# baaivision/Painter

Hardware: AMD Instinct MI355X
Metric: images/sec (896x448 pairs) ViT-L fwd+bwd (higher is better)
Workload: dtype bf16; 1 GPU; painter_vit_large_patch16_input896x448 bf16 batch=8/GPU fwd+bwd on 1xMI355X (BASELINE configs[1]); global_batch=8, image=896x448x3 stitched pair, mode=train (DropPath 0.1), parallelism=dp1, rccl_ranks=0, backend=n/a, grad_allreduce=n/a

## Files before the change

### include/painter_hip.h

```cpp
#ifndef PAINTER_HIP_H
#define PAINTER_HIP_H

#include <stdint.h>

#ifdef __cplusplus
extern "C" {
#endif

#ifndef __HIP__
typedef struct ihipStream_t* hipStream_t;
#endif

enum { PA_F32 = 0, PA_BF16 = 1 };
enum {
    PA_EPI_BIAS = 0,
    PA_EPI_BIAS_F32 = 1,
    PA_EPI_BIAS_GELU = 2,
    PA_EPI_BIAS_RESID = 3
};

#define PA_ABI_VERSION 8
int pa_abi_version(void);
int pa_debug_set(int which, int value);
int pa_debug_get(int which);

int pa_linear_fwd(int dtype, int epilogue, const void* x , int64_t ldx, const void* w ,
                  const float* bias , void* out, void* out2, int64_t ldo, const float* resid ,
                  const float* rowscale , int rows_per_sample, int M, int N, int K,
                  hipStream_t stream);
int pa_linear_fwd_skip(int dtype, int epilogue, const void* x, int64_t ldx, const void* w, const float* bias, void* out, void* out2,
                       int64_t ldo, const float* resid, const float* rowscale, int rows_per_sample, int M, int N, int K,
                       const float* rowskip, int skip_rows_per_sample, hipStream_t stream);
int pa_linear_pixshuf(int dtype, const void* x, int64_t ldx, const void* w , const float* bias,
                      void* out_nhwc, int batch, int Hp, int Wp, int P, int C, int K, hipStream_t stream);
int64_t pa_linear_dgrad_workspace_bytes(int M, int K);
int pa_linear_dgrad(int dtype, const void* dy , int64_t lddy, const void* w ,
                    const void* gelu_aux , void* dx , int64_t lddx, float* dx_colsum,
                    void* workspace, int M, int N, int K, hipStream_t stream);
int pa_linear_dgrad_skip(int dtype, const void* dy, int64_t lddy, const void* w, const void* gelu_aux, void* dx, int64_t lddx, float* dx_colsum,
                         void* workspace, int M, int N, int K, const float* rowskip , int skip_rows_per_sample,
                         hipStream_t stream);
int64_t pa_linear_wgrad_workspace_bytes(int dtype, int M, int N, int K);
int pa_linear_wgrad(int dtype, const void* dy , int64_t lddy, const void* x , int64_t ldx,
                    float* dw , void* workspace, int M, int N, int K, hipStream_t stream);
int64_t pa_colsum_workspace_bytes(int M, int N);
int pa_colsum(int dtype, const void* x , int64_t ld, int M, int N, float* out , void* workspace,
              hipStream_t stream);
int pa_slab_reduce(const float* in, float* out, int64_t n, int nz, int64_t stride, int accumulate, hipStream_t stream);

int pa_layernorm_fwd(int dtype, const float* x, int64_t ldx, const float* gamma, const float* beta, float eps,
                     void* y , int64_t ldy, float* mean, float* rstd,
                     int R, int D, hipStream_t stream);
int64_t pa_layernorm_bwd_workspace_bytes(int R, int D);
int pa_layernorm_bwd(int dtype, const void* dy, int64_t lddy, const float* x, int64_t ldx, const float* mean,
                     const float* rstd, const float* gamma, const float* dres, float* dx, int64_t lddx, void* dxT,
                     int64_t lddxT, const float* rowscale, int rows_per_sample, float* dgamma_dbeta, float* dxT_colsum,
                     void* workspace, int R, int D, hipStream_t stream);
// ... 250 lines not shown
```

### painter_amd/_lib.py

```python
import ctypes
import os
import re

HERE = os.path.dirname(os.path.abspath(__file__))
HEADER = os.path.join(os.path.dirname(HERE), "include", "painter_hip.h")
LIB_PATH = os.environ.get("PAINTER_AMD_LIB") or os.path.join(HERE, "lib", "libpainter_hip.so")

PA_F32, PA_BF16 = 0, 1
EPI_BIAS, EPI_BIAS_F32, EPI_BIAS_GELU, EPI_BIAS_RESID = 0, 1, 2, 3
(KNOB_G256_STAGGER, KNOB_G256_NOSTORE, KNOB_G256_ORDER, KNOB_WGRAD_TARGET, KNOB_G256_SHORT_TILES, KNOB_G256_ILV, KNOB_RELPOS_SPLITS,
 KNOB_ATTN3_FUSE, KNOB_ATTN_LIGHT_LAST, KNOB_CONV_WGRAD_GROUPS, KNOB_LN_BWD_VARIANT, KNOB_G256_PATCH, KNOB_G256_MIXED) = range(13)
KNOB_G256_MIXED_NFULL, KNOB_DROP_SKIP, KNOB_DECODER_ROWS, KNOB_COUNT = 14, 16, 17, 18

_CT = {"int": ctypes.c_int, "int64_t": ctypes.c_int64, "float": ctypes.c_float, "double": ctypes.c_double, "hipStream_t": ctypes.c_void_p}


def parse_header(path=HEADER):
    src = open(path).read()
    src = re.sub(r"/\*.*?\*/", " ", src, flags=re.S)
    src = re.sub(r"//[^\n]*", " ", src)
    protos = {}
    for m in re.finditer(r"\b(int64_t|int)\s+(pa_\w+)\s*\(([^)]*)\)\s*;", src):
        ret, name, args = m.group(1), m.group(2), m.group(3).strip()
        argtypes = []
        if args and args != "void":
            for a in args.split(","):
                a = a.strip()
                if "*" in a:
                    argtypes.append(ctypes.c_void_p)
                else:
                    t = a.replace("const", " ").split()[0]
                    argtypes.append(_CT[t])
        protos[name] = (_CT[ret], argtypes)
    return protos


class _Lib:
    def __init__(self):
        self._dll = None
        self._protos = parse_header()

    def load(self):
        if self._dll is None:
            if not os.path.exists(LIB_PATH):
                raise RuntimeError(
                    "painter_amd: %s is missing -- run `python -m painter_amd.build` (or __graft_entry__.build()). "
                    "There is no CPU / PyTorch fallback for the hot path." % LIB_PATH)
            import torch
            dll = ctypes.CDLL(LIB_PATH)
            for name, (ret, args) in self._protos.items():
                fn = getattr(dll, name)
                fn.restype = ret
                fn.argtypes = args
            want = int(re.search(r"#define\s+PA_ABI_VERSION\s+(\d+)", open(HEADER).read()).group(1))
            got = dll.pa_abi_version()
            if got != want:
                raise RuntimeError("painter_amd: %s has C ABI version %d, include/painter_hip.h declares %d -- rebuild it "
                                   "(python -m painter_amd.build --force)" % (LIB_PATH, got, want))
            self._dll = dll
        return self._dll

    def __getattr__(self, name):
        if name.startswith("_"):
            raise AttributeError(name)
        return getattr(self.load(), name)


lib = _Lib()


def check(err, what=""):
    if err != 0:
        raise RuntimeError("painter_hip: %s failed with hipError %d" % (what, err))
```

### painter_amd/csrc/common.h

```cpp
#pragma once
#include <hip/hip_runtime.h>
#include <stdint.h>
#include <cstdlib>

typedef __bf16 bf16;
typedef __attribute__((ext_vector_type(8))) __bf16 bf16x8;
typedef __attribute__((ext_vector_type(16))) float f32x16;

#define DEVI __device__ __forceinline__

template <typename T> struct TT;
template <> struct TT<float> {
    static constexpr int EPC = 4;
    static constexpr int BK = 32;
    static constexpr int KSTEPS = 2;
    static constexpr int SPF = 2;
    typedef uint4 Vec4;
};
template <> struct TT<bf16> {
    static constexpr int EPC = 8;
    static constexpr int BK = 64;
    static constexpr int KSTEPS = 4;
    static constexpr int SPF = 1;
    typedef uint2 Vec4;
// ... 51 lines not shown
    const uint32_t u = __builtin_bit_cast(uint32_t, v);
    const auto r = __builtin_amdgcn_permlane16_swap(u, u, false, false);
    return __builtin_bit_cast(float, (threadIdx.x & 16) ? r[0] : r[1]);
}
DEVI float lane_xor32(float v) {
    const uint32_t u = __builtin_bit_cast(uint32_t, v);
    const auto r = __builtin_amdgcn_permlane32_swap(u, u, false, false);
    return __builtin_bit_cast(float, (threadIdx.x & 32) ? r[0] : r[1]);
}
DEVI float quad_sum(float v) { v += lane_xor1(v); v += lane_xor2(v); return v; }
DEVI float row16_sum(float v) { v = quad_sum(v); v += lane_dpp<0x141>(v); v += lane_dpp<0x140>(v); return v; }
DEVI float wave_sum(float v) { v = row16_sum(v); v += lane_xor16(v); v += lane_xor32(v); return v; }
DEVI float wave_max(float v) {
    v = fmaxf(v, lane_xor1(v)); v = fmaxf(v, lane_xor2(v));
    v = fmaxf(v, lane_dpp<0x141>(v)); v = fmaxf(v, lane_dpp<0x140>(v));
    v = fmaxf(v, lane_xor16(v)); v = fmaxf(v, lane_xor32(v));
    return v;
}

enum Knob {
    KNOB_G256_STAGGER = 0,
    KNOB_G256_NOSTORE = 1,
    KNOB_G256_ORDER = 2,
    KNOB_WGRAD_TARGET = 3,
    KNOB_G256_SHORT_TILES = 4,
    KNOB_G256_ILV = 5,
    KNOB_RELPOS_SPLITS = 6,
    KNOB_ATTN3_FUSE = 7,
    KNOB_ATTN_LIGHT_LAST = 8,
    KNOB_CONV_WGRAD_GROUPS = 9,
    KNOB_LN_BWD_VARIANT = 10,
    KNOB_G256_PATCH = 11,
    KNOB_G256_MIXED = 12,
    KNOB_FREE_13 = 13,
    KNOB_G256_MIXED_NFULL = 14,
    KNOB_FREE_15 = 15,
    KNOB_DROP_SKIP = 16,
    KNOB_DECODER_ROWS = 17,
    KNOB_COUNT = 18
};
inline int g_knob[KNOB_COUNT] = {};
static inline bool drop_skip_on() {
    static const int env = [] { const char* v = getenv("PAINTER_AMD_DROP_SKIP"); return v ? atoi(v) : 1; }();
    return g_knob[KNOB_DROP_SKIP] == 1 ? false : (g_knob[KNOB_DROP_SKIP] == 2 ? true : env != 0);
}
static inline bool decoder_rows_on() {
    static const int env = [] { const char* v = getenv("PAINTER_AMD_DECODER_ROWS"); return v ? atoi(v) : 1; }();
    return g_knob[KNOB_DECODER_ROWS] == 1 ? false : (g_knob[KNOB_DECODER_ROWS] == 2 ? true : env != 0);
}

inline long long g_attn_counts[6] = {0, 0, 0, 0, 0, 0};

DEVI float gelu_f(float x) { return 0.5f * x * (1.0f + erff(x * 0.70710678118654752f)); }
DEVI float gelu_grad_f(float x) {
    const float cdf = 0.5f * (1.0f + erff(x * 0.70710678118654752f));
    const float pdf = 0.39894228040143268f * __expf(-0.5f * x * x);
    return cdf + x * pdf;
}

DEVI void gelu_parts(float x, float& cdf, float& pdf_unnorm) {
    const float z = fabsf(x) * 0.70710678118654752f;
    const float t = __builtin_amdgcn_rcpf(fmaf(0.3275911f, z, 1.0f));
    const float e = __builtin_amdgcn_exp2f(-0.72134752044448170f * x * x);
    float p = fmaf(1.061405429f, t, -1.453152027f);
    p = fmaf(p, t, 1.421413741f);
    p = fmaf(p, t, -0.284496736f);
    p = fmaf(p, t, 0.254829592f);
// ... 68 lines not shown
```

### painter_amd/csrc/gemm.hip

```cpp
#include <cstdlib>
#include "gemm_engine.h"
#include "gemm256.h"
#include "../../include/painter_hip.h"

template <typename OutT> struct EpiBias {
    OutT* out; size_t ldo; const float* bias; int M, N;
    DEVI void operator()(const f32x16 (&acc)[2][2], int ib, int jb, int lane, int) const {
        foreach_acc(acc, ib, jb, lane, [&](int i, int j, float v) {
            if (i < M && j < N) out[(size_t)i * ldo + j] = from_f<OutT>(v + (bias ? bias[j] : 0.f));
        });
    }
};
constexpr float G8_OFF = 0.13f, G8_SCALE = 255.f / 1.26f, G8_STEP = 1.26f / 255.f;
DEVI uint32_t g8_code(float g) { return min((uint32_t)fmaf(g, G8_SCALE, G8_OFF * G8_SCALE + 0.5f), 255u); }
DEVI float g8_value(uint32_t q) { return fmaf((float)q, G8_STEP, -G8_OFF); }
template <typename T> struct GeluAux { typedef T type; };
template <> struct GeluAux<bf16> { typedef unsigned char type; };
template <typename T> struct EpiBiasGelu {
    typename GeluAux<T>::type* aux; T* act; size_t ld; const float* bias; int M, N;
    DEVI void operator()(const f32x16 (&acc)[2][2], int ib, int jb, int lane, int) const {
        foreach_acc(acc, ib, jb, lane, [&](int i, int j, float v) {
            if (i < M && j < N) {
                const T p = from_f<T>(v + bias[j]);
                if constexpr (std::is_same<T, bf16>::value) {
// ... 173 lines not shown
    struct Row { uint2 p; };
    DEVI Col col(int) const { return Col{}; }
    DEVI Row row(int i, int j) const {
        Row r{make_uint2(0, 0)};
        if (i < M && j < N) r.p = *reinterpret_cast<const uint2*>(aux + (size_t)i * ld + j);
        return r;
    }
    DEVI void decode(const Row& r, float (&g)[8]) const {
#pragma unroll
        for (int e = 0; e < 8; ++e) g[e] = g8_value(((e < 4 ? r.p.x : r.p.y) >> (8 * (e & 3))) & 0xffu);
    }
    DEVI void store(int i, int j, float4 a, float4 b, const Col&, const Row& r, int) const {
        if (i >= M || j >= N) return;
        float g[8];
        decode(r, g);
        store8(out + (size_t)i * ld + j, make_float4(a.x * g[0], a.y * g[1], a.z * g[2], a.w * g[3]), make_float4(b.x * g[4], b.y * g[5], b.z * g[6], b.w * g[7]));
    }
};
struct Epi4DGeluCS : Epi4DGelu {
    float* part;
    DEVI void store_cs(int i, int j, float4 a, float4 b, const Col&, const Row& r, int, float (&cs)[8]) const {
        if (i >= M || j >= N) return;
        float g[8];
        decode(r, g);
        const uint4 pk = make_uint4(pack_bf16x2(a.x * g[0], a.y * g[1]), pack_bf16x2(a.z * g[2], a.w * g[3]),
                                    pack_bf16x2(b.x * g[4], b.y * g[5]), pack_bf16x2(b.z * g[6], b.w * g[7]));
        *reinterpret_cast<uint4*>(out + (size_t)i * ld + j) = pk;
        cs[0] = fmaf(a.x, g[0], cs[0]); cs[1] = fmaf(a.y, g[1], cs[1]); cs[2] = fmaf(a.z, g[2], cs[2]); cs[3] = fmaf(a.w, g[3], cs[3]);
        cs[4] = fmaf(b.x, g[4], cs[4]); cs[5] = fmaf(b.y, g[5], cs[5]); cs[6] = fmaf(b.z, g[6], cs[6]); cs[7] = fmaf(b.w, g[7], cs[7]);
    }
    DEVI void colsum_out(int prow, int j, const float (&cs)[8]) const {
        if (j >= N) return;
        float* o = part + (size_t)prow * N + j;
        *reinterpret_cast<float4*>(o) = make_float4(cs[0], cs[1], cs[2], cs[3]);
        *reinterpret_cast<float4*>(o + 4) = make_float4(cs[4], cs[5], cs[6], cs[7]);
    }
};
template <> struct g256::epi_colsum<Epi4DGeluCS> { static constexpr bool value = true; };
struct Epi4PixShuf {
    bf16* out; const float* bias; int Hp, Wp, P, C, M, N;
    typedef EpiCol8 Col;
    typedef EpiNone Row;
    DEVI Col col(int j) const { return load_col8(bias, j, N); }
    DEVI Row row(int, int) const { return Row{}; }
    DEVI void store(int i, int j, float4 a, float4 b, const Col& cc, const Row&, int) const {
        if (i >= M || j >= N) return;
        const int L = Hp * Wp;
        const int bb = i / L, l = i - bb * L, h = l / Wp, w = l - h * Wp;
        const int c = j % C, pq = j / C, q = pq % P, p = pq / P;
        const size_t y = (size_t)bb * Hp * P + h * P + p, x = (size_t)w * P + q;
        store8(out + (y * (size_t)(Wp * P) + x) * C + c, add4(a, cc.a), add4(b, cc.b));
    }
};
struct Epi4Slab {
    float* out; size_t ldo; size_t slab; int M, N;
    static constexpr int HI_OFF = 32;
    typedef EpiNone Col;
    typedef EpiNone Row;
    DEVI Col col(int) const { return Col{}; }
    DEVI Row row(int, int) const { return Row{}; }
    DEVI void store(int i, int j, float4 a, float4 b, const Col&, const Row&, int split) const {
        if (i >= M || j >= N) return;
        store44(out + (size_t)split * slab + (size_t)i * ldo + j, j, N, a, b);
    }
};

__global__ __launch_bounds__(256) void slab_reduce_kernel(const float* __restrict__ in, float* out, size_t n, int nz, size_t stride, int accumulate) {
    __shared__ float4 sh[16][17];
    const int cg = threadIdx.x & 15, zl = threadIdx.x >> 4;
    const size_t i = ((size_t)blockIdx.x * 16 + cg) * 4;
    float4 s = make_float4(0, 0, 0, 0);
    if (i < n) {
#pragma unroll 4
        for (int z = zl; z < nz; z += 16) {
            const float4 v = *reinterpret_cast<const float4*>(in + (size_t)z * stride + i);
            s.x += v.x; s.y += v.y; s.z += v.z; s.w += v.w;
        }
    }
    sh[zl][cg] = s;
    __syncthreads();
    if (zl == 0 && i < n) {
        float4 t = accumulate ? *reinterpret_cast<const float4*>(out + i) : make_float4(0, 0, 0, 0);
#pragma unroll
        for (int k = 0; k < 16; ++k) { const float4 v = sh[k][cg]; t.x += v.x; t.y += v.y; t.z += v.z; t.w += v.w; }
        *reinterpret_cast<float4*>(out + i) = t;
    }
}
__global__ void slab_reduce_wide_kernel(const float* __restrict__ in, float* out, size_t n, int nz, size_t stride, int accumulate) {
    const size_t i = ((size_t)blockIdx.x * blockDim.x + threadIdx.x) * 4;
    if (i >= n) return;
    float4 s = accumulate ? *reinterpret_cast<const float4*>(out + i) : make_float4(0, 0, 0, 0);
#pragma unroll 4
    for (int z = 0; z < nz; ++z) {
        const float4 v = *reinterpret_cast<const float4*>(in + (size_t)z * stride + i);
        s.x += v.x; s.y += v.y; s.z += v.z; s.w += v.w;
    }
    *reinterpret_cast<float4*>(out + i) = s;
}
__global__ __launch_bounds__(256) void slab_reduce2_kernel(const float* __restrict__ in, float* out0, float* out1, size_t n0, size_t n, int nz, size_t stride) {
    __shared__ float4 sh[16][17];
    const int cg = threadIdx.x & 15, zl = threadIdx.x >> 4;
    const size_t i = ((size_t)blockIdx.x * 16 + cg) * 4;
    float4 s = make_float4(0, 0, 0, 0);
    if (i < n) {
#pragma unroll 4
        for (int z = zl; z < nz; z += 16) {
            const float4 v = *reinterpret_cast<const float4*>(in + (size_t)z * stride + i);
            s.x += v.x; s.y += v.y; s.z += v.z; s.w += v.w;
        }
    }
    sh[zl][cg] = s;
    __syncthreads();
    if (zl == 0 && i < n) {
        float4 t = make_float4(0, 0, 0, 0);
#pragma unroll
        for (int k = 0; k < 16; ++k) { const float4 v = sh[k][cg]; t.x += v.x; t.y += v.y; t.z += v.z; t.w += v.w; }
        *reinterpret_cast<float4*>(i < n0 ? out0 + i : out1 + (i - n0)) = t;
    }
}
int pa_slab_reduce2(const float* in, float* out0, float* out1, int64_t n0, int64_t n, int nz, int64_t stride, hipStream_t st) {
    if (n <= 0) return 0;
    if (n % 4 || n0 % 4 || stride % 4 || (n > n0 && out1 == nullptr)) return (int)hipErrorInvalidValue;
    PA_LAUNCH(slab_reduce2_kernel, dim3((unsigned)((n / 4 + 15) / 16)), dim3(256), 0, st, in, out0, out1, (size_t)n0, (size_t)n, nz, (size_t)stride);
    LAUNCH_CHECK();
}
extern "C" int pa_slab_reduce(const float* in, float* out, int64_t n, int nz, int64_t stride, int accumulate, hipStream_t st) {
    if (n <= 0) return 0;
    if (n % 4 || stride % 4) return (int)hipErrorInvalidValue;
    if (nz <= 16 && n >= (1 << 18))
        PA_LAUNCH(slab_reduce_wide_kernel, dim3((unsigned)((n / 4 + 255) / 256)), dim3(256), 0, st, in, out, (size_t)n, nz, (size_t)stride, accumulate);
    else
        PA_LAUNCH(slab_reduce_kernel, dim3((unsigned)((n / 4 + 15) / 16)), dim3(256), 0, st, in, out, (size_t)n, nz, (size_t)stride, accumulate);
    LAUNCH_CHECK();
}

template <typename T> __global__ __launch_bounds__(256) void colsum_kernel(const T* __restrict__ x, size_t ld, int M, int N, int rows_per_chunk, float* __restrict__ part,
                                                                           const int* __restrict__ mcount = nullptr) {
    if (mcount != nullptr) M = min(M, *mcount);
    const int cl = threadIdx.x & 31, rl = threadIdx.x >> 5;
    const int c0 = (blockIdx.x * 32 + cl) * 8;
    const int r0 = blockIdx.y * rows_per_chunk, r1 = min(M, r0 + rows_per_chunk);
    float s[8] = {0, 0, 0, 0, 0, 0, 0, 0};
    if (c0 < N) {
#pragma unroll 4
        for (int r = r0 + rl; r < r1; r += 8) {
            const T* p = x + (size_t)r * ld + c0;
            if constexpr (sizeof(T) == 2) {
                const uint4 w = *reinterpret_cast<const uint4*>(p);
                s[0] += bf16_lo(w.x); s[1] += bf16_hi(w.x); s[2] += bf16_lo(w.y); s[3] += bf16_hi(w.y);
                s[4] += bf16_lo(w.z); s[5] += bf16_hi(w.z); s[6] += bf16_lo(w.w); s[7] += bf16_hi(w.w);
            } else {
// ... 102 lines not shown

template <typename T>
static int linear_pixshuf_t(const T* x, int64_t ldx, const T* w, const float* bias, T* out, int Bn, int Hp, int Wp,
                            int P, int C, int K, hipStream_t st) {
    const int M = Bn * Hp * Wp, N = P * P * C;
    if constexpr (std::is_same<T, bf16>::value) {
        if (g256::ok(M, N, K, false, false, ldx, K) && C % 8 == 0)
            return g256::launch<false, false>(x, ldx, w, K, Epi4PixShuf{out, bias, Hp, Wp, P, C, M, N}, M, N, K, 1, st);
    }
    OpN<T> A{x, (size_t)ldx, M, 0};
    OpN<T> B{w, (size_t)K, N, 0};
    return launch_gemm<T, 2, 2>(A, B, EpiPixShuf<T>{out, bias, Hp, Wp, P, C, M, N}, M, N, K, 1, 1, st);
}
extern "C" int pa_linear_pixshuf(int dtype, const void* x, int64_t ldx, const void* w, const float* bias, void* out_nhwc,
                                 int batch, int Hp, int Wp, int P, int C, int K, hipStream_t st) {
    if (K % 8) return (int)hipErrorInvalidValue;
    if (dtype == PA_BF16) return linear_pixshuf_t<bf16>((const bf16*)x, ldx, (const bf16*)w, bias, (bf16*)out_nhwc, batch, Hp, Wp, P, C, K, st);
    return linear_pixshuf_t<float>((const float*)x, ldx, (const float*)w, bias, (float*)out_nhwc, batch, Hp, Wp, P, C, K, st);
}

extern "C" int64_t pa_linear_dgrad_workspace_bytes(int M, int K) {
    const int64_t fast = (int64_t)2 * ((M + g256::BM_HALF - 1) / g256::BM_HALF) * K * sizeof(float);
    const int64_t slow = pa_colsum_workspace_bytes(M, K);
    return fast > slow ? fast : slow;
}
template <typename T>
static int linear_dgrad_t(const T* dy, int64_t lddy, const T* w, const typename GeluAux<T>::type* pre , T* dx, int64_t lddx, float* dx_colsum, float* ws, int M,
                          int N, int K, hipStream_t st, const float* rowskip = nullptr, int skip_rps = 1) {
    if constexpr (std::is_same<T, bf16>::value) {
        if (g256::ok(M, K, N, false, true, lddy, K)) {
            if (pre && dx_colsum) {
                Epi4DGeluCS ep;
                ep.out = dx; ep.aux = pre; ep.ld = (size_t)lddx; ep.M = M; ep.N = K; ep.part = ws;
                int e = rowskip ? g256::launch_skip<true>(dy, lddy, w, K, ep, M, K, N, st, rowskip, skip_rps) : g256::launch<false, true>(dy, lddy, w, K, ep, M, K, N, 1, st);
                if (e) return e;
                return pa_slab_reduce(ws, dx_colsum, K, 2 * g256::row_tiles_used(M, K, 1), K, 0, st);
            }
            if (pre) return g256::launch<false, true>(dy, lddy, w, K, Epi4DGelu{dx, pre, (size_t)lddx, M, K}, M, K, N, 1, st);
            int e = rowskip ? g256::launch_skip<true>(dy, lddy, w, K, Epi4Bias<bf16>{dx, (size_t)lddx, nullptr, M, K}, M, K, N, st, rowskip, skip_rps)
                            : g256::launch<false, true>(dy, lddy, w, K, Epi4Bias<bf16>{dx, (size_t)lddx, nullptr, M, K}, M, K, N, 1, st);
            if (e || dx_colsum == nullptr) return e;
            return pa_colsum(PA_BF16, dx, lddx, M, K, dx_colsum, ws, st);
        }
    }
    OpN<T> A{dy, (size_t)lddy, M, 0};
    OpT<T> B{w, (size_t)K, K, 0};
    int e;
    if (pre) e = launch_gemm<T, 2, 2>(A, B, EpiDGelu<T>{dx, pre, (size_t)lddx, M, K}, M, K, N, 1, 1, st);
    else e = launch_gemm<T, 2, 2>(A, B, EpiBias<T>{dx, (size_t)lddx, nullptr, M, K}, M, K, N, 1, 1, st);
    if (e || dx_colsum == nullptr) return e;
    return pa_colsum(std::is_same<T, bf16>::value ? PA_BF16 : PA_F32, dx, lddx, M, K, dx_colsum, ws, st);
}
extern "C" int pa_linear_dgrad_skip(int dtype, const void* dy, int64_t lddy, const void* w, const void* gelu_aux,
                                    void* dx, int64_t lddx, float* dx_colsum, void* workspace, int M, int N, int K,
                                    const float* rowskip, int skip_rows_per_sample, hipStream_t st) {
    if (N % 8 || K % 4) return (int)hipErrorInvalidValue;
    if (dx_colsum != nullptr && (workspace == nullptr || K % 8 || lddx % 8)) return (int)hipErrorInvalidValue;
    if (rowskip != nullptr && skip_rows_per_sample < 1) return (int)hipErrorInvalidValue;
    if (!drop_skip_on()) rowskip = nullptr;
    if (dtype == PA_BF16)
        return linear_dgrad_t<bf16>((const bf16*)dy, lddy, (const bf16*)w, (const unsigned char*)gelu_aux, (bf16*)dx, lddx, dx_colsum, (float*)workspace, M, N, K, st,
                                    rowskip, skip_rows_per_sample);
    return linear_dgrad_t<float>((const float*)dy, lddy, (const float*)w, (const float*)gelu_aux, (float*)dx, lddx, dx_colsum, (float*)workspace, M, N, K, st);
}
extern "C" int pa_linear_dgrad(int dtype, const void* dy, int64_t lddy, const void* w, const void* gelu_aux,
                               void* dx, int64_t lddx, float* dx_colsum, void* workspace, int M, int N, int K, hipStream_t st) {
    return pa_linear_dgrad_skip(dtype, dy, lddy, w, gelu_aux, dx, lddx, dx_colsum, workspace, M, N, K, nullptr, 1, st);
}
// ... 42 lines not shown
        }
    }
    OpT<T> A{dy, (size_t)lddy, N, 0};
    OpT<T> B{x, (size_t)ldx, K, 0};
    const int s = wgrad_splits(M, N, K, TT<T>::BK);
    if (s == 1) return launch_gemm<T, 2, 2>(A, B, EpiSlab{dw, (size_t)K, 0, N, K}, N, K, M, 1, 1, st);
    int e = launch_gemm<T, 2, 2>(A, B, EpiSlab{ws, (size_t)K, (size_t)N * K, N, K}, N, K, M, s, 1, st);
    if (e) return e;
    return pa_slab_reduce(ws, dw, (int64_t)N * K, s, (int64_t)N * K, 0, st);
}
extern "C" int pa_linear_wgrad(int dtype, const void* dy, int64_t lddy, const void* x, int64_t ldx, float* dw,
                               void* workspace, int M, int N, int K, hipStream_t st) {
    if (N % 4 || K % 4) return (int)hipErrorInvalidValue;
    if (dtype == PA_BF16) return linear_wgrad_t<bf16>((const bf16*)dy, lddy, (const bf16*)x, ldx, dw, (float*)workspace, M, N, K, st);
    return linear_wgrad_t<float>((const float*)dy, lddy, (const float*)x, ldx, dw, (float*)workspace, M, N, K, st);
}

extern "C" int pa_fill_dead_rows(void* x, int64_t pitch_bytes, int64_t row_bytes, const int* rowmap, int M, hipStream_t st);
extern "C" int pa_linear_dgrad_live(const void* dy, int64_t lddy, const void* w, void* dx, int64_t lddx, const int* live, const int* rowmap,
                                    const int* count, int M, int N, int K, hipStream_t st) {
    if (live == nullptr || rowmap == nullptr || count == nullptr || M < 8 || K % 8 || lddx % 8) return (int)hipErrorInvalidValue;
    if (!g256::ok(M, K, N, false, true, lddy, K)) return (int)hipErrorInvalidValue;
    int e = pa_fill_dead_rows(dx, lddx * 2, (int64_t)K * 2, rowmap, M, st);
    if (e) return e;
    return g256::launch_live<false, true>((const bf16*)dy, lddy, (const bf16*)w, K, Epi4Scatter{(bf16*)dx, (size_t)lddx, live, count, M, K}, M, K, N, count, st);
}
extern "C" int pa_linear_wgrad_live(const void* dy, int64_t lddy, const void* x, int64_t ldx, float* dw, const int* count, int M, int N, int K,
                                    hipStream_t st) {
    if (count == nullptr || M < 128 || M % 128) return (int)hipErrorInvalidValue;
    if (!wgrad_fast(PA_BF16, M, N, K) || !g256::ok(N, K, M, true, true, lddy, ldx)) return (int)hipErrorInvalidValue;
    return g256::launch_live<true, true>((const bf16*)dy, lddy, (const bf16*)x, ldx, Epi4Slab{dw, (size_t)K, 0, N, K}, N, K, M, count, st);
}

extern "C" int pa_abi_version(void) { return PA_ABI_VERSION; }
extern "C" int pa_debug_get(int which) {
    return which < 0 || which >= KNOB_COUNT ? -1 : g_knob[which];
}
extern "C" int pa_debug_set(int which, int value) {
    if (which < 0 || which >= KNOB_COUNT) return (int)hipErrorInvalidValue;
    g_knob[which] = value;
    return 0;
}
```

### painter_amd/csrc/gemm256.h

```cpp
#pragma once
#include "common.h"
#include <cstdlib>
#include <type_traits>

namespace g256 {

constexpr int BM = 256, BN = 256, BK = 64, NT = 512;
constexpr int LDS_BYTES = 131072;
typedef __attribute__((address_space(3))) void lds_void;
typedef __attribute__((address_space(1))) const void gbl_cvoid;

DEVI constexpr int unit_off(bool isB, int sub, int stage) { return (isB ? 65536 : 0) + sub * 32768 + stage * 16384; }

template <int N> DEVI void wait_vm() { asm volatile("s_waitcnt vmcnt(%0)" ::"n"(N) : "memory"); }
DEVI void wait_lgkm0() { asm volatile("s_waitcnt lgkmcnt(0)" ::: "memory"); }

template <bool MM, bool IS_A>
DEVI uint32_t src_off(int tid, int j, int sub, int tile0, int rows, uint32_t ld) {
    const int cidx = j * NT + tid;
    if constexpr (!MM) {
        const int u = cidx >> 3, p = cidx & 7;
        const int kc = p ^ ((u >> 1) & 7);
        int row = IS_A ? ((u >> 6) * 128 + sub * 64 + (u & 63)) : ((u >> 5) * 64 + sub * 32 + (u & 31));
        row = min(tile0 + row, rows - 1);
        return ((uint32_t)row * ld + kc * 8) * 2u;
    } else {
        const int k = cidx >> 4, cp = cidx & 15;
        const int c = cp ^ (4 * (k & 3));
        int n = IS_A ? ((c >> 3) * 128 + sub * 64 + (c & 7) * 8) : ((c >> 2) * 64 + sub * 32 + (c & 3) * 8);
        n = min(tile0 + n, rows - 8);
        return ((uint32_t)k * ld + n) * 2u;
    }
}

// ... 19 lines not shown
        lds_read128<IMM>(q0, base[0]);
        lds_read128<IMM>(q1, base[1]);
        lds_read128<IMM>(q2, base[2]);
        lds_read128<IMM>(q3, base[3]);
    }
    template <int KS> DEVI bf16x8 k() const {
        return __builtin_bit_cast(bf16x8, KS == 0 ? q0 : KS == 1 ? q1 : KS == 2 ? q2 : q3);
    }
};
template <> struct Frag4<true> {
    uint2 l0, h0, l1, h1, l2, h2, l3, h3;
    template <int IMM> DEVI void read(const uint32_t (&base)[4], int which_mb) {
        const uint32_t b = base[which_mb];
        lds_read64_tr<IMM + 0 * 4096>(l0, b);
        lds_read64_tr<IMM + 0 * 4096 + 1024>(h0, b);
        lds_read64_tr<IMM + 1 * 4096>(l1, b);
        lds_read64_tr<IMM + 1 * 4096 + 1024>(h1, b);
        lds_read64_tr<IMM + 2 * 4096>(l2, b);
        lds_read64_tr<IMM + 2 * 4096 + 1024>(h2, b);
        lds_read64_tr<IMM + 3 * 4096>(l3, b);
        lds_read64_tr<IMM + 3 * 4096 + 1024>(h3, b);
    }
    template <int KS> DEVI bf16x8 k() const {
        typedef __attribute__((ext_vector_type(2))) uint32_t u2;
        typedef __attribute__((ext_vector_type(4))) uint32_t u4;
        const uint2 l = KS == 0 ? l0 : KS == 1 ? l1 : KS == 2 ? l2 : l3;
        const uint2 h = KS == 0 ? h0 : KS == 1 ? h1 : KS == 2 ? h2 : h3;
        u2 lv = {l.x, l.y}, hv = {h.x, h.y};
        return __builtin_bit_cast(bf16x8, __builtin_shufflevector(lv, hv, 0, 1, 2, 3));
    }
};

template <class Epi> struct epi_colsum { static constexpr bool value = false; };
template <class Epi, class = void> struct epi_hi_off { static constexpr int value = 4; };
template <class Epi> struct epi_hi_off<Epi, std::void_t<decltype(Epi::HI_OFF)>> { static constexpr int value = Epi::HI_OFF; };
constexpr int BM_SHORT = 224;
constexpr int BM_HALF = 128;
template <bool AMM, bool BMM, int ILV, class Epi, bool SHORT = false, bool MIXED = false, bool SKIP = false, bool LIVE = false>
__global__ __launch_bounds__(NT) void gemm256_kernel(const bf16* __restrict__ Ag, uint32_t lda, const bf16* __restrict__ Bg,
                                                      uint32_t ldb, Epi epi, int M, int N, int ktiles, int ktiles_per_split,
                                                      int tiles_n, int stagger, int order, int nfull, int patch,
                                                      const float* __restrict__ rowskip, int rps, const int* __restrict__ live_count) {
    static_assert(!(LIVE && (SHORT || MIXED || SKIP)), "a device-side count goes with uniform 256-row tiles");
    static_assert(!(SHORT && AMM), "the 224-row tile is built for a K-major A operand");
    static_assert(!(SKIP && AMM), "row tiles are skipped only for a K-major A operand");
    static_assert(!(MIXED && (AMM || SHORT)), "half tiles are built for a K-major A operand and 256-row full tiles");
    constexpr int BMR = SHORT ? BM_SHORT : BM;
    extern __shared__ __attribute__((aligned(1024))) unsigned char smem[];
    const int tid = threadIdx.x, lane = tid & 63;
    if (stagger > 0 && blockIdx.x < 256 && blockIdx.y == 0) {
        const int64_t wait = ((int64_t)stagger * (((blockIdx.x >> 3) * 5) & 15)) >> 4;
        const uint64_t t0 = __builtin_amdgcn_s_memtime();
        while ((int64_t)(__builtin_amdgcn_s_memtime() - t0) < wait) __builtin_amdgcn_s_sleep(16);
    }
    const int wv = __builtin_amdgcn_readfirstlane(tid >> 6);
    const int wr = wv >> 2, wc = wv & 3;

    const bool htile = MIXED && (int)blockIdx.x >= nfull * tiles_n;
    int nwg = MIXED ? (htile ? (int)gridDim.x - nfull * tiles_n : nfull * tiles_n) : (int)gridDim.x;
    if constexpr (LIVE) {
        if constexpr (AMM) {
            ktiles = ktiles_per_split = min(ktiles, ((*live_count + 127) >> 7) * 2);
        } else {
            M = min(M, *live_count);
            nwg = ((M + BM - 1) / BM) * tiles_n;
            if ((int)blockIdx.x >= nwg) return;
// ... 308 lines not shown
                const int mb = hf * 2 + m2;
                if (SHORT && mb == 3 && !blk3) continue;
#pragma unroll
                for (int nb = 0; nb < 2; ++nb)
#pragma unroll
                    for (int q = 0; q < 4; ++q) {
                        const f32x16& c = acc[mb][nb];
                        *reinterpret_cast<float4*>(stg + lr * 68 + nb * 32 + q * 8 + g * 4) =
                            make_float4(c[q * 4 + 0], c[q * 4 + 1], c[q * 4 + 2], c[q * 4 + 3]);
                    }
                const int ib = rbase + (mb >> 1) * 64 + (mb & 1) * 32;
#pragma unroll
                for (int st = 0; st < 4; ++st) {
                    const int r = st * 8 + rrow;
                    const float4 lo = *reinterpret_cast<const float4*>(stg + r * 68 + c0);
                    const float4 hi = *reinterpret_cast<const float4*>(stg + r * 68 + c0 + HO);
                    if constexpr (epi_colsum<Epi>::value) epi.store_cs(ib + r, jcol, lo, hi, col, rows[m2][st], split, cs);
                    else epi.store(ib + r, jcol, lo, hi, col, rows[m2][st], split);
                }
            }
        }
        if constexpr (epi_colsum<Epi>::value) {
#pragma unroll
            for (int e = 0; e < 8; ++e) {
                float v = cs[e];
                v += lane_dpp<0x128>(v);
                v += lane_xor16(v);
                v += lane_xor32(v);
                cs[e] = v;
            }
            if (lane < 8) epi.colsum_out((htile ? nfull + tm : tm) * 2 + wr, jcol, cs);
        }
    }
}

static inline int per_split(int ktiles, int nsplit) {
    int per = (ktiles + nsplit - 1) / nsplit;
    return per + (per & 1);
}
template <bool AMM, bool BMM, int ILV, bool SHORT, class Epi, bool MIXED = false, bool SKIP = false, bool LIVE = false>
static int launch_ilv(const bf16* A, size_t lda, const bf16* B, size_t ldb, Epi epi, int M, int N, int K, int nsplit, hipStream_t st, int nfull = 0,
                      const float* rowskip = nullptr, int rps = 1, const int* live_count = nullptr);
#ifndef G256_ILV_DEFAULT
#define G256_ILV_DEFAULT 2
#endif
static inline bool use_short(int M, int N, int nsplit, bool amm) {
    if (amm || nsplit != 1 || M < BM) return false;
    if (g_knob[KNOB_G256_SHORT_TILES] == 1) return false;
    if (g_knob[KNOB_G256_SHORT_TILES] == 2) return true;
    static const int cost = [] { const char* v = getenv("PA_G256_SHORT_COST"); return v ? atoi(v) : 92; }();
    const int tiles_n = (N + BN - 1) / BN;
    const long t256 = (long)((M + BM - 1) / BM) * tiles_n, t224 = (long)((M + BM_SHORT - 1) / BM_SHORT) * tiles_n;
    const long r256 = (t256 + 255) / 256 * 100, r224 = (t224 + 255) / 256 * cost;
    return r224 < r256;
}
struct TilePlan { bool is_short, mixed; int nfull; };
static inline TilePlan tile_plan(int M, int N, int nsplit, bool amm) {
    TilePlan p{use_short(M, N, nsplit, amm), false, 0};
    if (amm || nsplit != 1 || M < 2 * BM || g_knob[KNOB_G256_MIXED] == 1 || g_knob[KNOB_G256_SHORT_TILES] != 0) return p;
    if (g_knob[KNOB_G256_MIXED] == 2 && g_knob[KNOB_G256_MIXED_NFULL] > 0 && (long)g_knob[KNOB_G256_MIXED_NFULL] * BM < M) return TilePlan{false, true, g_knob[KNOB_G256_MIXED_NFULL]};
    static const int cs = [] { const char* v = getenv("PA_G256_SHORT_COST"); return v ? atoi(v) : 97; }();
    static const int ch = [] { const char* v = getenv("PA_G256_HALF_COST"); return v ? atoi(v) : 75; }();
    const int tn = (N + BN - 1) / BN;
    auto rounds = [](long t) { return (t + 255) / 256; };
    long best = p.is_short ? rounds((long)((M + BM_SHORT - 1) / BM_SHORT) * tn) * cs : rounds((long)((M + BM - 1) / BM) * tn) * 100;
    for (int r = 1; r <= 64; ++r) {
// ... 82 lines not shown
```

### painter_amd/ops.py

```python
import torch

from ._lib import (EPI_BIAS, EPI_BIAS_F32, EPI_BIAS_GELU, EPI_BIAS_RESID, KNOB_DECODER_ROWS, KNOB_DROP_SKIP, PA_BF16, PA_F32, check, lib)

_WS = {}


def stream():
    return torch.cuda.current_stream().cuda_stream


def code(dtype):
    if dtype == torch.bfloat16:
        return PA_BF16
    if dtype == torch.float32:
        return PA_F32
    raise TypeError("painter_amd supports float32 / bfloat16 operand types, got %s" % dtype)


def p(t):
    return 0 if t is None else t.data_ptr()


def workspace(nbytes, device, slot=0):
    key = (device, slot, torch.cuda.current_stream(device).cuda_stream)
    buf = _WS.get(key)
    if buf is None or buf.numel() < nbytes:
        buf = torch.empty(max(int(nbytes), 1 << 20), dtype=torch.uint8, device=device)
        _WS[key] = buf
    return buf


def _mbs(mask_u8):
    return 0 if mask_u8.shape[0] == 1 else mask_u8.stride(0)


def _knob(which, mode):
    old = int(lib.pa_debug_get(which))
    if mode is not None:
        check(lib.pa_debug_set(which, int(mode)), "pa_debug_set")
    return old


def _req(t, dtype=None):
    assert t.is_cuda and t.stride(-1) == 1, "device tensor with unit inner stride required"
    if dtype is not None:
        assert t.dtype == dtype, (t.dtype, dtype)
    return t


def _skip_args(rowskip, skip_rows_per_sample, M):
    if rowskip is None:
        return 0, 1
    assert rowskip.dtype == torch.float32 and rowskip.is_cuda and rowskip.is_contiguous() and skip_rows_per_sample >= 1
    assert rowskip.numel() * skip_rows_per_sample >= M, (rowskip.numel(), skip_rows_per_sample, M)
    return rowskip.data_ptr(), int(skip_rows_per_sample)


def drop_skip(mode=None):
    return _knob(KNOB_DROP_SKIP, mode)


def linear_fwd(x, w, bias, epilogue=EPI_BIAS, out=None, out2=None, resid=None, rowscale=None, rows_per_sample=1, *, rowskip=None,
               skip_rows_per_sample=None):
    M, K = x.shape
    N = w.shape[0]
    T = x.dtype
    _req(x); _req(w, T)
    assert w.is_contiguous() and w.shape[1] == K
    if out is None:
        odt = torch.float32 if epilogue in (EPI_BIAS_F32, EPI_BIAS_RESID) else T
        out = torch.empty((M, N), dtype=odt, device=x.device)
    if epilogue == EPI_BIAS_RESID:
        assert resid is not None and resid.dtype == torch.float32 and resid.stride(0) == out.stride(0)
    sk, srps = _skip_args(rowskip, rows_per_sample if skip_rows_per_sample is None else skip_rows_per_sample, M)
    check(lib.pa_linear_fwd_skip(code(T), epilogue, p(x), x.stride(0), p(w), p(bias), p(out), p(out2), out.stride(0),
                                 p(resid), p(rowscale), rows_per_sample, M, N, K, sk, srps, stream()), "pa_linear_fwd_skip")
    return out


def linear_gelu(x, w, bias, need_aux=True, *, rowskip=None, rows_per_sample=1):
    M = x.shape[0]
    N = w.shape[0]
    act = torch.empty((M, N), dtype=x.dtype, device=x.device)
    aux = torch.empty((M, N), dtype=gelu_aux_dtype(x.dtype), device=x.device) if need_aux else None
    assert aux is None or aux.stride(0) == act.stride(0)
    linear_fwd(x, w, bias, EPI_BIAS_GELU, out=act, out2=aux, rowskip=rowskip, skip_rows_per_sample=rows_per_sample)
    return act, aux


G8_OFF, G8_RANGE = 0.13, 1.26


# ... 478 lines not shown
```

Before: 165.1 images/sec.

## Fuse dgrad GELU column-sum reduction into GEMM via last-block arrival counters

```diff
diff --git a/include/painter_hip.h b/include/painter_hip.h
--- a/include/painter_hip.h
+++ b/include/painter_hip.h
@@ -23,6 +23,9 @@
 int pa_abi_version(void);
 int pa_debug_set(int which, int value);
 int pa_debug_get(int which);
+int pa_reduce_counters_reset(hipStream_t stream);
+int pa_reduce_counters_launches(hipStream_t stream);
+int pa_reduce_counters_nonzero(hipStream_t stream);
 
 int pa_linear_fwd(int dtype, int epilogue, const void* x , int64_t ldx, const void* w ,
                   const float* bias , void* out, void* out2, int64_t ldo, const float* resid ,
diff --git a/painter_amd/_lib.py b/painter_amd/_lib.py
--- a/painter_amd/_lib.py
+++ b/painter_amd/_lib.py
@@ -10,7 +10,7 @@
 EPI_BIAS, EPI_BIAS_F32, EPI_BIAS_GELU, EPI_BIAS_RESID = 0, 1, 2, 3
 (KNOB_G256_STAGGER, KNOB_G256_NOSTORE, KNOB_G256_ORDER, KNOB_WGRAD_TARGET, KNOB_G256_SHORT_TILES, KNOB_G256_ILV, KNOB_RELPOS_SPLITS,
  KNOB_ATTN3_FUSE, KNOB_ATTN_LIGHT_LAST, KNOB_CONV_WGRAD_GROUPS, KNOB_LN_BWD_VARIANT, KNOB_G256_PATCH, KNOB_G256_MIXED) = range(13)
-KNOB_G256_MIXED_NFULL, KNOB_DROP_SKIP, KNOB_DECODER_ROWS, KNOB_COUNT = 14, 16, 17, 18
+KNOB_TWO_LAUNCH_REDUCE, KNOB_G256_MIXED_NFULL, KNOB_DROP_SKIP, KNOB_DECODER_ROWS, KNOB_COUNT = 13, 14, 16, 17, 18
 
 _CT = {"int": ctypes.c_int, "int64_t": ctypes.c_int64, "float": ctypes.c_float, "double": ctypes.c_double, "hipStream_t": ctypes.c_void_p}
 
@@ -71,4 +71,9 @@
 
 def check(err, what=""):
     if err != 0:
+        try:
+            import torch
+            lib.pa_reduce_counters_reset(torch.cuda.current_stream().cuda_stream)
+        except Exception:
+            pass
         raise RuntimeError("painter_hip: %s failed with hipError %d" % (what, err))
diff --git a/painter_amd/csrc/common.h b/painter_amd/csrc/common.h
--- a/painter_amd/csrc/common.h
+++ b/painter_amd/csrc/common.h
@@ -107,7 +107,7 @@
     KNOB_LN_BWD_VARIANT = 10,
     KNOB_G256_PATCH = 11,
     KNOB_G256_MIXED = 12,
-    KNOB_FREE_13 = 13,
+    KNOB_TWO_LAUNCH_REDUCE = 13,
     KNOB_G256_MIXED_NFULL = 14,
     KNOB_FREE_15 = 15,
     KNOB_DROP_SKIP = 16,
diff --git a/painter_amd/csrc/gemm.hip b/painter_amd/csrc/gemm.hip
--- a/painter_amd/csrc/gemm.hip
+++ b/painter_amd/csrc/gemm.hip
@@ -229,11 +229,21 @@
     DEVI void colsum_out(int prow, int j, const float (&cs)[8]) const {
         if (j >= N) return;
         float* o = part + (size_t)prow * N + j;
+        if (cnt != nullptr) {
+            inl::store_wt(o, make_float4(cs[0], cs[1], cs[2], cs[3]));
+            inl::store_wt(o + 4, make_float4(cs[4], cs[5], cs[6], cs[7]));
+            return;
+        }
         *reinterpret_cast<float4*>(o) = make_float4(cs[0], cs[1], cs[2], cs[3]);
         *reinterpret_cast<float4*>(o + 4) = make_float4(cs[4], cs[5], cs[6], cs[7]);
     }
+    int* cnt; float* colsum;
+    DEVI void colsum_finish(int j0, int nrows, float4* lds, int tid) const {
+        inl::finish_cols256<g256::NT>(part, (size_t)N, nrows, colsum, (size_t)j0, (size_t)N, lds, tid);
+    }
 };
 template <> struct g256::epi_colsum<Epi4DGeluCS> { static constexpr bool value = true; };
+template <> struct g256::epi_finish<Epi4DGeluCS> { static constexpr bool value = true; };
 struct Epi4PixShuf {
     bf16* out; const float* bias; int Hp, Wp, P, C, M, N;
     typedef EpiCol8 Col;
@@ -263,57 +273,27 @@
 };
 
 __global__ __launch_bounds__(256) void slab_reduce_kernel(const float* __restrict__ in, float* out, size_t n, int nz, size_t stride, int accumulate) {
-    __shared__ float4 sh[16][17];
+    __shared__ float4 sh[16 * 17];
     const int cg = threadIdx.x & 15, zl = threadIdx.x >> 4;
     const size_t i = ((size_t)blockIdx.x * 16 + cg) * 4;
-    float4 s = make_float4(0, 0, 0, 0);
-    if (i < n) {
-#pragma unroll 4
-        for (int z = zl; z < nz; z += 16) {
-            const float4 v = *reinterpret_cast<const float4*>(in + (size_t)z * stride + i);
-            s.x += v.x; s.y += v.y; s.z += v.z; s.w += v.w;
-        }
-    }
-    sh[zl][cg] = s;
-    __syncthreads();
-    if (zl == 0 && i < n) {
-        float4 t = accumulate ? *reinterpret_cast<const float4*>(out + i) : make_float4(0, 0, 0, 0);
-#pragma unroll
-        for (int k = 0; k < 16; ++k) { const float4 v = sh[k][cg]; t.x += v.x; t.y += v.y; t.z += v.z; t.w += v.w; }
-        *reinterpret_cast<float4*>(out + i) = t;
-    }
+    const bool live = i < n;
+    const float4 t0 = (accumulate && zl == 0 && live) ? *reinterpret_cast<const float4*>(out + i) : make_float4(0, 0, 0, 0);
+    const float4 t = inl::sum_strided16<1, 17>(in + i, stride, nz, cg, zl, live, sh, t0);
+    if (zl == 0 && live) *reinterpret_cast<float4*>(out + i) = t;
 }
 __global__ void slab_reduce_wide_kernel(const float* __restrict__ in, float* out, size_t n, int nz, size_t stride, int accumulate) {
     const size_t i = ((size_t)blockIdx.x * blockDim.x + threadIdx.x) * 4;
     if (i >= n) return;
-    float4 s = accumulate ? *reinterpret_cast<const float4*>(out + i) : make_float4(0, 0, 0, 0);
-#pragma unroll 4
-    for (int z = 0; z < nz; ++z) {
-        const float4 v = *reinterpret_cast<const float4*>(in + (size_t)z * stride + i);
-        s.x += v.x; s.y += v.y; s.z += v.z; s.w += v.w;
-    }
-    *reinterpret_cast<float4*>(out + i) = s;
+    const float4 s = accumulate ? *reinterpret_cast<const float4*>(out + i) : make_float4(0, 0, 0, 0);
+    *reinterpret_cast<float4*>(out + i) = inl::sum_ascending(s, nz, [&](int z) { return *reinterpret_cast<const float4*>(in + (size_t)z * stride + i); });
 }
 __global__ __launch_bounds__(256) void slab_reduce2_kernel(const float* __restrict__ in, float* out0, float* out1, size_t n0, size_t n, int nz, size_t stride) {
-    __shared__ float4 sh[16][17];
+    __shared__ float4 sh[16 * 17];
     const int cg = threadIdx.x & 15, zl = threadIdx.x >> 4;
     const size_t i = ((size_t)blockIdx.x * 16 + cg) * 4;
-    float4 s = make_float4(0, 0, 0, 0);
-    if (i < n) {
-#pragma unroll 4
-        for (int z = zl; z < nz; z += 16) {
-            const float4 v = *reinterpret_cast<const float4*>(in + (size_t)z * stride + i);
-            s.x += v.x; s.y += v.y; s.z += v.z; s.w += v.w;
-        }
-    }
-    sh[zl][cg] = s;
-    __syncthreads();
-    if (zl == 0 && i < n) {
-        float4 t = make_float4(0, 0, 0, 0);
-#pragma unroll
-        for (int k = 0; k < 16; ++k) { const float4 v = sh[k][cg]; t.x += v.x; t.y += v.y; t.z += v.z; t.w += v.w; }
-        *reinterpret_cast<float4*>(i < n0 ? out0 + i : out1 + (i - n0)) = t;
-    }
+    const bool live = i < n;
+    const float4 t = inl::sum_strided16<1, 17>(in + i, stride, nz, cg, zl, live, sh, make_float4(0, 0, 0, 0));
+    if (zl == 0 && live) *reinterpret_cast<float4*>(i < n0 ? out0 + i : out1 + (i - n0)) = t;
 }
 int pa_slab_reduce2(const float* in, float* out0, float* out1, int64_t n0, int64_t n, int nz, int64_t stride, hipStream_t st) {
     if (n <= 0) return 0;
@@ -482,8 +462,10 @@
             if (pre && dx_colsum) {
                 Epi4DGeluCS ep;
                 ep.out = dx; ep.aux = pre; ep.ld = (size_t)lddx; ep.M = M; ep.N = K; ep.part = ws;
+                ep.cnt = inl::counters(st, (K + g256::BN - 1) / g256::BN);
+                ep.colsum = dx_colsum;
                 int e = rowskip ? g256::launch_skip<true>(dy, lddy, w, K, ep, M, K, N, st, rowskip, skip_rps) : g256::launch<false, true>(dy, lddy, w, K, ep, M, K, N, 1, st);
-                if (e) return e;
+                if (e || ep.cnt != nullptr) return e;
                 return pa_slab_reduce(ws, dx_colsum, K, 2 * g256::row_tiles_used(M, K, 1), K, 0, st);
             }
             if (pre) return g256::launch<false, true>(dy, lddy, w, K, Epi4DGelu{dx, pre, (size_t)lddx, M, K}, M, K, N, 1, st);
@@ -592,6 +574,35 @@
     return g256::launch_live<true, true>((const bf16*)dy, lddy, (const bf16*)x, ldx, Epi4Slab{dw, (size_t)K, 0, N, K}, N, K, M, count, st);
 }
 
+extern "C" int pa_reduce_counters_reset(hipStream_t st) {
+    std::lock_guard<std::mutex> lock(inl::g_ring_mutex);
+    int dev = 0;
+    PA_TRY(hipGetDevice(&dev));
+    auto it = inl::g_rings.find({dev, st});
+    if (it == inl::g_rings.end()) return 0;
+    return (int)hipMemsetAsync(it->second.dev, 0, (size_t)inl::RING_SLICES * inl::SLICE_INTS * sizeof(int), st);
+}
+extern "C" int pa_reduce_counters_launches(hipStream_t st) {
+    std::lock_guard<std::mutex> lock(inl::g_ring_mutex);
+    int dev = 0;
+    if (hipGetDevice(&dev) != hipSuccess) return 0;
+    auto it = inl::g_rings.find({dev, st});
+    return it == inl::g_rings.end() ? 0 : (int)(it->second.next & 0x7fffffffu);
+}
+extern "C" int pa_reduce_counters_nonzero(hipStream_t st) {
+    std::lock_guard<std::mutex> lock(inl::g_ring_mutex);
+    int dev = 0;
+    if (int e = (int)hipGetDevice(&dev)) return -e;
+    auto it = inl::g_rings.find({dev, st});
+    if (it == inl::g_rings.end()) return 0;
+    std::vector<int> host((size_t)inl::RING_SLICES * inl::SLICE_INTS);
+    if (int e = (int)hipStreamSynchronize(st)) return -e;
+    if (int e = (int)hipMemcpy(host.data(), it->second.dev, host.size() * sizeof(int), hipMemcpyDeviceToHost)) return -e;
+    int n = 0;
+    for (int v : host) n += v != 0;
+    return n;
+}
+
 extern "C" int pa_abi_version(void) { return PA_ABI_VERSION; }
 extern "C" int pa_debug_get(int which) {
     return which < 0 || which >= KNOB_COUNT ? -1 : g_knob[which];
diff --git a/painter_amd/csrc/gemm256.h b/painter_amd/csrc/gemm256.h
--- a/painter_amd/csrc/gemm256.h
+++ b/painter_amd/csrc/gemm256.h
@@ -1,5 +1,6 @@
 #pragma once
 #include "common.h"
+#include "inlaunch.h"
 #include <cstdlib>
 #include <type_traits>
 
@@ -85,6 +86,7 @@
 };
 
 template <class Epi> struct epi_colsum { static constexpr bool value = false; };
+template <class Epi> struct epi_finish { static constexpr bool value = false; };
 template <class Epi, class = void> struct epi_hi_off { static constexpr int value = 4; };
 template <class Epi> struct epi_hi_off<Epi, std::void_t<decltype(Epi::HI_OFF)>> { static constexpr int value = Epi::HI_OFF; };
 constexpr int BM_SHORT = 224;
@@ -459,6 +461,13 @@
             if (lane < 8) epi.colsum_out((htile ? nfull + tm : tm) * 2 + wr, jcol, cs);
         }
     }
+    if constexpr (epi_finish<Epi>::value) {
+        if (epi.cnt != nullptr) {
+            int* const flag = reinterpret_cast<int*>(smem + LDS_BYTES - 16);
+            const int tiles_m = (int)gridDim.x / tiles_n;
+            if (inl::arrive<true>(epi.cnt + tn, tiles_m, flag)) epi.colsum_finish(j0, 2 * tiles_m, reinterpret_cast<float4*>(smem), tid);
+        }
+    }
 }
 
 static inline int per_split(int ktiles, int nsplit) {
diff --git a/painter_amd/csrc/inlaunch.h b/painter_amd/csrc/inlaunch.h
--- /dev/null
+++ b/painter_amd/csrc/inlaunch.h
@@ -0,0 +1,105 @@
+#pragma once
+#include "common.h"
+#include <map>
+#include <mutex>
+#include <utility>
+#include <vector>
+
+namespace inl {
+
+template <class F> DEVI float4 sum_ascending(float4 s, int nz, F&& load) {
+#pragma unroll 4
+    for (int z = 0; z < nz; ++z) {
+        const float4 v = load(z);
+        s.x += v.x; s.y += v.y; s.z += v.z; s.w += v.w;
+    }
+    return s;
+}
+template <int ZPT, int PITCH> DEVI float4 sum_strided16(const float* in, size_t stride, int nz, int cg, int zq, bool live, float4* sh, float4 t) {
+#pragma unroll
+    for (int k = 0; k < ZPT; ++k) {
+        const int zl = zq + k * (16 / ZPT);
+        float4 s = make_float4(0, 0, 0, 0);
+        if (live) {
+#pragma unroll 4
+            for (int z = zl; z < nz; z += 16) {
+                const float4 v = *reinterpret_cast<const float4*>(in + (size_t)z * stride);
+                s.x += v.x; s.y += v.y; s.z += v.z; s.w += v.w;
+            }
+        }
+        sh[zl * PITCH + cg] = s;
+    }
+    __syncthreads();
+    if (zq == 0 && live) {
+#pragma unroll
+        for (int k = 0; k < 16; ++k) { const float4 v = sh[k * PITCH + cg]; t.x += v.x; t.y += v.y; t.z += v.z; t.w += v.w; }
+    }
+    return t;
+}
+constexpr int FIN_SH = 16 * 64;
+template <int NTHREADS> DEVI void finish_cols256(const float* in, size_t stride, int nz, float* out, size_t col0, size_t n, float4* sh, int tid) {
+    constexpr int ZPT = 1024 / NTHREADS;
+    const int cg = tid & 63, zq = tid >> 6;
+    const size_t i = col0 + (size_t)cg * 4;
+    const bool live = i < n;
+    const float4 t = sum_strided16<ZPT, 64>(in + i, stride, nz, cg, zq, live, sh, make_float4(0, 0, 0, 0));
+    if (zq == 0 && live) *reinterpret_cast<float4*>(out + i) = t;
+}
+
+DEVI void store_wt(float* p, float v) { __hip_atomic_store(p, v, __ATOMIC_RELAXED, __HIP_MEMORY_SCOPE_AGENT); }
+DEVI void store_wt(float* p, float4 v) {
+    u64* q = reinterpret_cast<u64*>(p);
+    __hip_atomic_store(q, (u64)__builtin_bit_cast(uint32_t, v.x) | ((u64)__builtin_bit_cast(uint32_t, v.y) << 32), __ATOMIC_RELAXED, __HIP_MEMORY_SCOPE_AGENT);
+    __hip_atomic_store(q + 1, (u64)__builtin_bit_cast(uint32_t, v.z) | ((u64)__builtin_bit_cast(uint32_t, v.w) << 32), __ATOMIC_RELAXED, __HIP_MEMORY_SCOPE_AGENT);
+}
+template <bool WT> DEVI bool arrive(int* counter, int expected, int* flag) {
+    asm volatile("s_waitcnt vmcnt(0)" ::: "memory");
+    __syncthreads();
+    if (threadIdx.x == 0) {
+        if constexpr (!WT) {
+            __builtin_amdgcn_fence(__ATOMIC_RELEASE, "agent");
+            asm volatile("s_waitcnt vmcnt(0)" ::: "memory");
+        }
+        const int ticket = __hip_atomic_fetch_add(counter, 1, __ATOMIC_RELAXED, __HIP_MEMORY_SCOPE_AGENT);
+        const int last = ticket == expected - 1;
+        if (last) {
+            __hip_atomic_store(counter, 0, __ATOMIC_RELAXED, __HIP_MEMORY_SCOPE_AGENT);
+            __builtin_amdgcn_fence(__ATOMIC_ACQUIRE, "agent");
+            asm volatile("s_waitcnt vmcnt(0)" ::: "memory");
+        }
+        *flag = last;
+    }
+    __syncthreads();
+    return *flag != 0;
+}
+
+constexpr int RING_SLICES = 4, SLICE_INTS = 1024;
+struct Ring { int* dev; unsigned next; };
+inline std::mutex g_ring_mutex;
+inline std::map<std::pair<int, hipStream_t>, Ring> g_rings;
+static inline bool inlaunch_on() {
+    static const int env = [] { const char* v = getenv("PAINTER_AMD_INLAUNCH_REDUCE"); return v ? atoi(v) : 1; }();
+    return g_knob[KNOB_TWO_LAUNCH_REDUCE] == 1 ? false : (g_knob[KNOB_TWO_LAUNCH_REDUCE] == 2 ? true : env != 0);
+}
+static inline Ring* ring_of(hipStream_t st) {
+    int dev = 0;
+    if (hipGetDevice(&dev) != hipSuccess) return nullptr;
+    auto it = g_rings.find({dev, st});
+    if (it != g_rings.end()) return &it->second;
+    hipStreamCaptureStatus cap = hipStreamCaptureStatusNone;
+    if (hipStreamIsCapturing(st, &cap) != hipSuccess || cap != hipStreamCaptureStatusNone) return nullptr;
+    int* d = nullptr;
+    const size_t bytes = (size_t)RING_SLICES * SLICE_INTS * sizeof(int);
+    if (hipMalloc(&d, bytes) != hipSuccess) { (void)hipGetLastError(); return nullptr; }
+    if (hipMemset(d, 0, bytes) != hipSuccess || hipDeviceSynchronize() != hipSuccess) { (void)hipGetLastError(); (void)hipFree(d); return nullptr; }
+    return &(g_rings[{dev, st}] = Ring{d, 0u});
+}
+static inline int* counters(hipStream_t st, int n) {
+    if (!inlaunch_on() || n < 1 || n > SLICE_INTS) return nullptr;
+    std::lock_guard<std::mutex> lock(g_ring_mutex);
+    Ring* r = ring_of(st);
+    if (r == nullptr) return nullptr;
+    return r->dev + (size_t)(r->next++ % RING_SLICES) * SLICE_INTS;
+}
+
+}
diff --git a/painter_amd/ops.py b/painter_amd/ops.py
--- a/painter_amd/ops.py
+++ b/painter_amd/ops.py
@@ -1,6 +1,7 @@
 import torch
 
-from ._lib import (EPI_BIAS, EPI_BIAS_F32, EPI_BIAS_GELU, EPI_BIAS_RESID, KNOB_DECODER_ROWS, KNOB_DROP_SKIP, PA_BF16, PA_F32, check, lib)
+from ._lib import (EPI_BIAS, EPI_BIAS_F32, EPI_BIAS_GELU, EPI_BIAS_RESID, KNOB_DECODER_ROWS, KNOB_DROP_SKIP, KNOB_TWO_LAUNCH_REDUCE, PA_BF16, PA_F32, check,
+                   lib)
 
 _WS = {}
 
@@ -58,6 +59,16 @@
 
 def drop_skip(mode=None):
     return _knob(KNOB_DROP_SKIP, mode)
+
+
+def inlaunch_reduce(mode=None):
+    return _knob(KNOB_TWO_LAUNCH_REDUCE, mode)
+
+
+def reduce_counters_nonzero():
+    n = int(lib.pa_reduce_counters_nonzero(stream()))
+    check(-n if n < 0 else 0, "pa_reduce_counters_nonzero")
+    return n
 
 
 def linear_fwd(x, w, bias, epilogue=EPI_BIAS, out=None, out2=None, resid=None, rowscale=None, rows_per_sample=1, *, rowskip=None,
```

Result: no change. 164.8 images/sec (-0.2%).
